# konstantineder/montecarlo-risk-engine

Hardware: AMD Instinct MI355X
Metric: path-steps/sec at 1M paths x 250 steps; PV/CVA rel-error vs CPU ref (higher is better)
Workload: dtype f64

## Files before the change

### montecarlo-risk-engine_amd/csrc/kf_lean.hip

```cpp
#include <cstdlib>
#include <map>
#include <utility>

#include "kf_common.h"

namespace {

template <int NSLOT, int PPL>
__device__ __forceinline__ void lean_date_cva(const FastDateCvaLds* __restrict__ rp, const double (&reg)[PPL][2 * NSLOT], double (&cva)[PPL],
                                              const double* __restrict__ etab)
{
    const mcx_expq_coef ec = mcx_expq_load(mcx_region_zero());
    const FastDateCvaLds r = *rp;
    double xe[2 * PPL], ev[2 * PPL];
#pragma unroll
    for (int q = 0; q < PPL; ++q) {
        xe[2 * q] = fma(r.m_s1, reg[q][FDC_S_REG], fma(r.m_n1, reg[q][FDC_NI_REG], r.m_c0));
        xe[2 * q + 1] = fma(r.c_c1, reg[q][FDC_C_REG], r.c_c0);
    }
    mcx_exp_tab_n<2 * PPL>(xe, ev, etab, ec);
#pragma unroll
    for (int q = 0; q < PPL; ++q) {
        const double x = fma(r.x_d, reg[q][FDC_X_REG], r.x_a);
        double p = 0.0;
        p += fma(fma(r.row0[2], x, r.row0[1]), x, r.row0[0]);
        p += fma(fma(r.row1[2], x, r.row1[1]), x, r.row1[0]);
        const double w = r.m_b * ev[2 * q];
        const double cs = fma(r.c_b, ev[2 * q + 1], r.c_a);
        cva[q] = fma(fmax(p, 0.0), w * (1.0 - cs), cva[q]);
    }
}

#define MCX_LEAN_WAVES 4
template <int NSLOT, int NZ, bool INJECT, int SIG, int PPL, bool SIMULATE, int DK = 0>
__global__ __launch_bounds__(MCX_BLOCK, MCX_LEAN_WAVES) void kf_lean(const FusedArgs)
{
    static_assert(DK == 0 || (SIG == SIG_VAS_CIR_E && SIMULATE && !INJECT), "the cva-date kernel simulates the Vasicek + CIR++ signature");
    constexpr int NREG = 2 * NSLOT;
    constexpr int TILE = MCX_BLOCK * PPL;
    extern __shared__ double lds[];
    KArgs& a0 = kargs_region(0);
    const int n_rec = a0.n_rec;
    const int64_t n = a0.k1.n;
    for (int q = threadIdx.x; q < 9 * n_rec; q += MCX_BLOCK) lds[q] = 0.0;
    FastDateCvaLds* const dlds = (FastDateCvaLds*)(lds + ((9 * n_rec + 1) & ~1));
    if constexpr (DK == 1) {
        const FastDateCva* __restrict__ dc = a0.cva_dates;
        const double* __restrict__ cf = a0.coeffs;
        const int n_dates = a0.n_dates;
        for (int q = threadIdx.x; q < 16 * n_dates; q += MCX_BLOCK) {
            const int t = q >> 4, e = q & 15;
            double v;
            if (e < FDC_HEAD) {
                v = ((const double*)(dc + t))[e];
            } else {
                const int off = e < FDC_HEAD + 3 ? dc[t].coeff_off0 : dc[t].coeff_off1;
                v = off >= 0 ? cf[off + (e - FDC_HEAD) % 3] : 0.0;
            }
            ((double*)dlds)[q] = v;
        }
    }
    constexpr int BMB = SIG == SIG_VAS_CIR_E ? 10 : 7;
    constexpr int BM = (INJECT || !SIMULATE) ? 0 : MCX_BM_LDS_DOUBLES_B(BMB);
    __shared__ double tab_lds[BM + MCX_EXP_LDS_DOUBLES];
    const double* tab = nullptr;
    const double* etab = tab_lds + BM;
    mcx_exp_tab_load(tab_lds + BM);
    if (BM) { mcx_bm_load<BMB>(tab_lds); tab = tab_lds; }
    __syncthreads();
    const int64_t tiles = (n + TILE - 1) / TILE;
    double n_block = 0.0;

    for (int64_t tile = blockIdx.x; tile < tiles; tile += gridDim.x) {
        const bool first_tile = tile == (int64_t)blockIdx.x;
        int64_t i[PPL];
        bool live[PPL];
        uint64_t path[PPL];
        double reg[PPL][NREG];
        double cfs[PPL], cva[PPL];
        int est[PPL];
        int n_init, n_steps;
        {
            KArgs& a = kargs_region(mcx_region_zero());
            const auto& k = a.k1;
#pragma unroll
            for (int q = 0; q < PPL; ++q) {
                const int64_t i_raw = tile * TILE + q * MCX_BLOCK + threadIdx.x;
                live[q] = i_raw < n;
                i[q] = live[q] ? i_raw : n - 1;
                path[q] = k.path_offset + (uint64_t)i[q];
                sim_init_state<NSLOT, SIG>(k, reg[q]);
                cfs[q] = 0.0; cva[q] = 0.0;
                est[q] = a.init_state[0];
            }
            const int64_t rest = n - tile * TILE;
            n_block += (double)(rest < TILE ? rest : TILE);
            n_init = k.n_initial_store; n_steps = k.n_steps;
        }
        if (SIMULATE) {
        int step = 0, t_init = 0;
#pragma unroll 1
        while (true) {
            const bool init = t_init < n_init;
            if (!init && step >= n_steps) break;
            int st = init ? t_init : -1;
            t_init += init ? 1 : 0;
            {
                const int zr0 = mcx_region_zero();
                const auto& k = kargs_region(zr0).k1;
                const uint64_t seed = k.seed;
                const mcx_bm_coef bc = mcx_bm_coef_load(zr0);
                const mcx_bm_vconst vc = mcx_bm_vconst_make<BMB>(bc);
#pragma unroll 1
                while (st < 0 && step < n_steps) {
                    if constexpr (SIG == SIG_GENERIC) {
#pragma unroll
                        for (int q = 0; q < PPL; ++q) sim_substep<NSLOT, NZ, INJECT, SIG, BMB, true>(k, step, path[q], i[q], reg[q], tab, seed, bc, &vc);
                        st = ldk(&k.steps[step].store_idx);
                    } else {
                        double zz[PPL][NZ], uu[PPL];
                        bool rare = false;
                        const StepData<NSLOT, NZ> sdat = sim_step_load<NSLOT, NZ, SIG>(k, step);
                        __builtin_amdgcn_sched_barrier(0);
                        if constexpr (INJECT) {
#pragma unroll
                            for (int q = 0; q < PPL; ++q) sim_draw<NZ, true, SIG, BMB>(k, step, path[q], i[q], zz[q], uu[q], tab, seed, bc, &vc);
                        } else {
                            uint32_t st_q[PPL];
#pragma unroll
                            for (int q = 0; q < PPL; ++q) st_q[q] = (uint32_t)step;
                            rare = sim_draw_n<PPL, NZ, SIG, BMB>(k, st_q, path, zz, uu, tab, seed, bc, vc);
                        }
                        if (!INJECT && __builtin_expect(__any(rare), 0)) {
#pragma unroll
                            for (int q = 0; q < PPL; ++q) sim_draw<NZ, false, SIG, BMB, true>(k, step, path[q], i[q], zz[q], uu[q], tab, seed, bc, &vc);
                        }
#pragma unroll
                        for (int q = 0; q < PPL; ++q) st = sim_apply_loaded<NSLOT, NZ, SIG, true>(k, sdat, reg[q], zz[q], uu[q]);
                    }
                    ++step;
                }
            }
            if (st >= 0) {
                if constexpr (DK == 1) lean_date_cva<NSLOT, PPL>(dlds + st, reg, cva, etab);
                else lean_date<NSLOT, SIG, PPL, true>(st, i, live, first_tile, lds, reg, cfs, cva, est, etab);
            }
        }
        } else {
            auto load_row = [&](int t, double (&dst)[PPL][NREG]) {
                const auto& k = kargs_region(0).k1;
                const int D = k.n_state;
#pragma unroll
                for (int q = 0; q < PPL; ++q)
#pragma unroll
                    for (int sl = 0; sl < NSLOT; ++sl) {
                        const bool bs = sig_kind(SIG, sl) >= 0 ? sig_is_bs(SIG, sl) : (k.slots[sl].kind == MCX_MODEL_BS);
                        const int c = k.slots[sl].state_off;
                        dst[q][2 * sl] = k.paths[((int64_t)t * D + c) * k.ld + i[q]];
                        dst[q][2 * sl + 1] = bs ? 0.0 : k.paths[((int64_t)t * D + c + 1) * k.ld + i[q]];
                    }
            };
            const int n_dates = kargs_region(0).n_dates;
            double bufb[PPL][NREG];
            load_row(0, reg);
            load_row(n_dates > 1 ? 1 : 0, bufb);
#pragma unroll 1
            for (int t = 0; t < n_dates; t += 2) {
                lean_date<NSLOT, SIG, PPL, false>(t, i, live, first_tile, lds, reg, cfs, cva, est, etab);
                if (t + 2 < n_dates) load_row(t + 2, reg);
                if (t + 1 < n_dates) {
                    lean_date<NSLOT, SIG, PPL, false>(t + 1, i, live, first_tile, lds, bufb, cfs, cva, est, etab);
                    if (t + 3 < n_dates) load_row(t + 3, bufb);
                }
            }
        }
        {
            KArgs& a = kargs_region(mcx_region_zero());
#pragma unroll
            for (int q = 0; q < PPL; ++q) if (a.cfs && live[q]) a.cfs[i[q]] = cfs[q];
            if (a.rec_pv[0] >= 0) lean_record<PPL>(cfs, live, a.rec_pv[0], n_rec, first_tile, lds);
            if (a.rec_cva[0] >= 0) {
                const double lgd = a.lgd[0];
                double cc[PPL];
#pragma unroll
                for (int q = 0; q < PPL; ++q) cc[q] = cva[q] * lgd;
                lean_record<PPL>(cc, live, a.rec_cva[0], n_rec, first_tile, lds);
            }
        }
    }
    __syncthreads();
    for (int r = threadIdx.x; r < n_rec; r += MCX_BLOCK) {
        double s1 = 0.0, s2 = 0.0;
        for (int w = 0; w < 4; ++w) { s1 += lds[n_rec + (w * n_rec + r) * 2]; s2 += lds[n_rec + (w * n_rec + r) * 2 + 1]; }
        double* dst = a0.partials + ((int64_t)blockIdx.x * n_rec + r) * 4;
        dst[0] = n_block; dst[1] = lds[r]; dst[2] = s1; dst[3] = s2;
    }
}

template <int NSLOT, int NZ, int SIG, int PPL>
int launch_lean_shape(const FusedArgs& a, int n_cu, bool inject, bool simulate, hipStream_t s)
{
    const int64_t tiles = (a.k1.n + MCX_BLOCK * PPL - 1) / (MCX_BLOCK * PPL);
    const size_t lds = sizeof(double) * (size_t)((9 * a.n_rec + 1) & ~1);
    const size_t lds_cva = lds + sizeof(FastDateCvaLds) * (size_t)a.n_dates;
    auto residency = [&](auto kernel, size_t bytes) {
        thread_local std::map<std::pair<const void*, size_t>, int> cache;
        const auto key = std::make_pair((const void*)kernel, bytes);
        auto it = cache.find(key);
        if (it == cache.end()) {
            int per_cu = 0;
            if (hipOccupancyMaxActiveBlocksPerMultiprocessor(&per_cu, kernel, MCX_BLOCK, bytes) != hipSuccess || per_cu < 1) per_cu = 1;
            it = cache.emplace(key, per_cu < MCX_LEAN_WAVES ? per_cu : MCX_LEAN_WAVES).first;
        }
        return (int64_t)it->second * n_cu;
    };
    auto sized = [&](int64_t resident) {
        if (tiles <= resident) return (int)tiles;
        const int64_t per = (tiles + resident - 1) / resident;
// ... 79 lines not shown
```

### montecarlo-risk-engine_amd/csrc/mcx_device.h

```cpp
#pragma once
#include "mcx_internal.h"

struct K1Args {
    mcx_slot slots[MCX_MAX_SLOTS];
    double init_state[MCX_MAX_STATE];
    const mcx_step* __restrict__ steps;
    const double* __restrict__ chol;
    const double* __restrict__ aux;
    double* __restrict__ paths;
    const double* __restrict__ inject_z;
    const double* __restrict__ inject_u;
    const double* __restrict__ init_paths;
    int64_t n, ld;
    uint64_t seed, path_offset;
    int32_t scheme, n_steps, n_state, n_initial_store, flags, n_uniform;
};

static inline void mcx_fill_k1_args(const mcx_sim* sim, uint64_t seed, uint64_t path_offset, int64_t n_paths, int64_t ld,
                                    double* d_paths, const double* d_inject_z, const double* d_inject_u, K1Args* a)
{
    const mcx_sim_desc& d = sim->desc;
    memset(a, 0, sizeof(*a));
    for (int s = 0; s < d.n_slots; ++s) a->slots[s] = d.slots[s];
    for (int c = 0; c < d.n_state; ++c) a->init_state[c] = d.init_state[c];
    a->steps = sim->d_steps; a->chol = sim->d_chol; a->aux = sim->d_aux;
    a->paths = d_paths; a->inject_z = d_inject_z; a->inject_u = d_inject_u;
    a->n = n_paths; a->ld = ld; a->seed = seed; a->path_offset = path_offset;
    a->scheme = d.scheme; a->n_steps = d.n_steps; a->n_state = d.n_state; a->n_initial_store = d.n_initial_store;
    a->flags = d.flags; a->n_uniform = d.n_uniform;
}

__device__ __forceinline__ void philox4x32_10(uint32_t c0, uint32_t c1, uint32_t c2, uint32_t c3, uint32_t k0, uint32_t k1,
                                              uint32_t& o0, uint32_t& o1, uint32_t& o2, uint32_t& o3)
{
#pragma unroll
    for (int r = 0; r < 10; ++r) {
        const uint64_t p0 = (uint64_t)0xD2511F53u * c0;
        const uint64_t p1 = (uint64_t)0xCD9E8D57u * c2;
        const uint32_t n0 = __builtin_amdgcn_bitop3_b32((uint32_t)(p1 >> 32), c1, k0, 0x96);
        const uint32_t n2 = __builtin_amdgcn_bitop3_b32((uint32_t)(p0 >> 32), c3, k1, 0x96);
        c1 = (uint32_t)p1;
        c3 = (uint32_t)p0;
        c0 = n0;
        c2 = n2;
        k0 += 0x9E3779B9u;
        k1 += 0xBB67AE85u;
    }
    o0 = c0; o1 = c1; o2 = c2; o3 = c3;
}

__device__ __forceinline__ double u53(uint32_t lo, uint32_t hi, const mcx_bm_vconst* vc = nullptr)
{
    if (vc) return fma((double)hi, vc->s32, fma((double)(lo >> 11), vc->s53, vc->c54));
    return fma((double)hi, 0x1.0p-32, fma((double)(lo >> 11), 0x1.0p-53, 0x1.0p-54));
}

struct DevBridge {
    uint64_t seed, path_offset;
    const double* const* inject;
    int64_t ld;
};

__device__ __forceinline__ double dev_barrier_event(const DevEvent& e, const DevTerm* __restrict__ terms, const double* __restrict__ coeffs,
                                                    const DevBridge* __restrict__ bridge, const double* __restrict__ paths, int64_t D,
                                                    int64_t ld, int64_t i, double num)
{
    const int types = (int)e.aux[3];
    const int t1 = types & 7, t2 = types >> 3;
    const bool with_bridge = e.aux[0] == 5.0;
    double mx = -1.0e300, mn = 1.0e300, keep1 = 1.0, keep2 = 1.0, prev1 = 0.0, prev2 = 0.0;
    double c = 0.0;
    int draw_id = 0;
    DevBridge br = {0, 0, nullptr, 0};
    const double* __restrict__ inj = nullptr;
    if (with_bridge) {
        c = ldk(coeffs + e.coeff_off);
        draw_id = (int)ldk(coeffs + e.coeff_off + 1);
        br = ldk_struct(bridge);
        if (br.inject) inj = br.inject[draw_id];
    }
    AtomCache bc = {-1, -1, 0.0};
    for (int j = e.term_begin; j < e.term_end; ++j) {
        const double s = dev_atom_cached(ldk_struct(&terms[j]).atom, paths, D, ld, i, bc);
        mx = fmax(mx, s); mn = fmin(mn, s);
        if (with_bridge) {
            const double cur1 = mcx_log(s / e.aux[1]), cur2 = t2 ? mcx_log(s / e.aux[2]) : 0.0;
            if (j > e.term_begin) {
                const int k = j - e.term_begin - 1;
                for (int bi = 0; bi < (t2 ? 2 : 1); ++bi) {
                    const double p = mcx_exp(c * (bi ? prev2 * cur2 : prev1 * cur1));
                    double u;
                    if (inj) u = inj[(int64_t)(2 * k + bi) * br.ld + i];
                    else {
                        uint32_t w0, w1, w2, w3;
                        const uint64_t path = br.path_offset + (uint64_t)i;
                        philox4x32_10((uint32_t)path, (uint32_t)(path >> 32), (uint32_t)k, 0x80000000u | (uint32_t)(2 * draw_id + bi),
                                      (uint32_t)br.seed, (uint32_t)(br.seed >> 32), w0, w1, w2, w3);
                        u = u53(w0, w1);
                    }
                    const double hit = fmin(fmax((p - u + 0.05) / 0.1, 0.0), 1.0);
                    if (bi) keep2 *= 1.0 - hit; else keep1 *= 1.0 - hit;
                }
            }
            prev1 = cur1; prev2 = cur2;
        }
    }
    double pay = fmax(e.sign * (dev_atom(e.x, paths, D, ld, i) - e.strike), 0.0) * dev_barrier_ind(t1, e.aux[1], mx, mn);
    if (with_bridge) pay *= (t1 <= 2) ? keep1 : 1.0 - keep1;
    if (t2) {
        pay *= dev_barrier_ind(t2, e.aux[2], mx, mn);
        if (with_bridge) pay *= (t2 <= 2) ? keep2 : 1.0 - keep2;
    }
    return pay / num;
}

template <bool TAB = false, int BMB = 7, bool GUARD = true>
__device__ __forceinline__ bool pair_from_words(uint32_t w0, uint32_t w1, uint32_t w2, uint32_t w3, double& ua, double& z0, double& z1,
                                                const double* __restrict__ tab, const mcx_bm_coef& bc, const mcx_bm_vconst* vc = nullptr)
{
    ua = u53(w0, w1, vc);
    double s, c, r;
    if (TAB) {
        const double r2 = mcx_m2log_tab<BMB>(ua, tab, bc, vc);
        if (!GUARD) r = mcx_sqrt_gp(r2);
        else if (__builtin_expect(__any(w1 == 0xffffffffu), 0)) r = ua < 1.0 ? mcx_sqrt_g(r2) : 0.0;
        else r = mcx_sqrt_gp(r2);
        const int j = (int)(w3 >> (32 - BMB));
        const double ur = u53(w2, w3 & ((1u << (32 - BMB)) - 1u), vc);
        mcx_sincos2pi_tab<BMB>(ur, j, tab, s, c, bc, vc);
    } else {
        r = mcx_sqrt(-2.0 * mcx_log(ua));
        mcx_sincos2pi(u53(w2, w3), s, c);
    }
    z0 = r * c;
    z1 = r * s;
    return w1 == 0xffffffffu;
}

template <bool TAB = false, int BMB = 7, bool GUARD = true>
__device__ __forceinline__ bool draw_pair(uint64_t seed, uint64_t path, uint32_t step, uint32_t draw, double& ua, double& z0, double& z1,
                                          const double* __restrict__ tab, const mcx_bm_coef& bc, const mcx_bm_vconst* vc = nullptr)
{
    uint32_t w0, w1, w2, w3;
    philox4x32_10((uint32_t)path, (uint32_t)(path >> 32), step, draw, (uint32_t)seed, (uint32_t)(seed >> 32), w0, w1, w2, w3);
    return pair_from_words<TAB, BMB, GUARD>(w0, w1, w2, w3, ua, z0, z1, tab, bc, vc);
}

template <bool TAB = false>
__device__ __forceinline__ void draw_pair(uint64_t seed, uint64_t path, uint32_t step, uint32_t draw, double& ua, double& z0, double& z1,
                                          const double* __restrict__ tab = nullptr)
{
    const mcx_bm_coef bc = mcx_bm_coef_load();
    draw_pair<TAB>(seed, path, step, draw, ua, z0, z1, tab, bc);
}

__device__ __forceinline__ double degree_of_truth(double x, bool fuzzy, double eps)
{
    if (!fuzzy) return x > 0.0 ? 1.0 : 0.0;
    const double v = (x + eps) / (2.0 * eps);
    return fmin(fmax(v, 0.0), 1.0);
}

struct AuxPtr {
    const double* __restrict__ p;
    __device__ __forceinline__ double operator[](int i) const { return ldk(p + i); }
    __device__ __forceinline__ mcx_aux_drv drv() const { return ldk_struct((const mcx_aux_drv*)(p + MCX_AUX_C0)); }
};
struct AuxRegs {
    double v[MCX_AUX];
    __device__ __forceinline__ double operator[](int i) const { return v[i]; }
    __device__ __forceinline__ mcx_aux_drv drv() const { mcx_aux_drv d; d.c0 = v[MCX_AUX_C0]; d.c1 = v[MCX_AUX_C1]; d.c2 = v[MCX_AUX_C2]; return d; }
};

template <int KIND, int SCHEME, bool POS = false, class SL, class AUX>
__device__ __forceinline__ void step_slot(const SL& sl, int scheme_rt, int flags, double dt, double sq,
                                          const AUX& aux, double& s0, double& s1, double zc0, double zc1, double u)
{
    const auto* p = sl.p;
    const int scheme = SCHEME >= 0 ? SCHEME : scheme_rt;
    switch (KIND >= 0 ? KIND : sl.kind) {
    case MCX_MODEL_BS:
        if (scheme == MCX_SCHEME_ANALYTICAL) {
            s0 = s0 * mcx_exp(aux[0] + (zc0 - aux[1]));
        } else {
            const mcx_aux_drv dc = aux.drv();
            s0 = fma(s0, fma(dc.c2, zc0, dc.c0), s0);
        }
        break;
    case MCX_MODEL_VASICEK: {
        const double r = s0;
        s1 = s1 + r * dt;
        if (scheme == MCX_SCHEME_ANALYTICAL) s0 = (p[2] + (r - p[2]) * aux[0]) + zc0;
        else {
            const mcx_aux_drv dc = aux.drv();
            s0 = fma(dc.c1, r, s0);
            s0 = fma(dc.c2, zc0, s0);
            s0 = s0 + dc.c0;
        }
        break;
    }
    case MCX_MODEL_HW: {
        const double r = s0;
        s1 = s1 + r * dt;
        if (scheme == MCX_SCHEME_ANALYTICAL) s0 = r * aux[0] + aux[1] + zc0;
        else s0 = r + (aux[0] - p[3] * r) * dt + p[1] * sq * zc0;
        break;
    }
    case MCX_MODEL_CIRPP: {
        const double y = s0;
        const double sy = POS ? mcx_sqrt_gp(y) : mcx_sqrt_g(y);
        const mcx_aux_drv dc = aux.drv();
        s1 = fma(y + aux[0], dt, s1);
        s0 = fma(dc.c1, y, s0);
        s0 = fma(dc.c2 * sy, zc0, s0);
        s0 = s0 + dc.c0;
        s0 = fmax(s0, 1e-12);
        break;
    }
    case MCX_MODEL_CIRPP_DET:
        s1 = s1 + aux[0] * dt;
        s0 = aux[1];
        break;
    case MCX_MODEL_S2F: {
        const double x = s0, y = s1;
        if (scheme == MCX_SCHEME_ANALYTICAL) {
            s0 = x * aux[0] + zc0;
            s1 = y + p[3] * dt + zc1;
        } else {
            s0 = x - p[1] * x * dt + p[2] * sq * zc0;
            s1 = y + p[3] * dt + p[4] * sq * zc1;
        }
        break;
    }
    case MCX_MODEL_HESTON: {
        const double logS = s0, v = s1;
        const double sigma = p[1], rate = p[2], kappa = p[4], theta = p[5];
        if (scheme == MCX_SCHEME_EULER) {
            const double sv = mcx_sqrt(fmax(v, 0.0));
            s0 = logS + (rate - 0.5 * v) * dt + sv * sq * zc0;
            s1 = fmax(v + kappa * (theta - v) * dt + sigma * sv * sq * zc1, 0.0);
        } else {
            const double eps = 1e-12;
            const bool fuzzy = (flags & MCX_FLAG_SMOOTHING) != 0;
            const double m = theta + (v - theta) * aux[0];
            const double s2 = v * aux[6] + aux[7];
            const double omu = fmax(1.0 - u, eps);
            const double d1 = m * m + eps, d5 = m + eps;
            const double d15 = d1 * d5;
            const double ra = mcx_rcp(d15 * omu);
            const double r_omu = ra * d15, ra6 = ra * omu;
            const double r1 = ra6 * d5, r5 = ra6 * d1;
            const double psi = s2 * r1;
            const double d2 = psi + eps, d4 = psi + 1.0;
            const double rb = mcx_rcp(d2 * d4);
            const double invpsi = rb * d4, r4 = rb * d2;
            const double t = fmax(2.0 * invpsi - 1.0, 0.0);
            double root = mcx_sqrt_g(2.0 * invpsi * t);
            root = invpsi < 0.0 ? __builtin_nan("") : root;
            const double b2u = 2.0 * invpsi - 1.0 + root;
            const double b2 = b2u < 0.0 ? 0.0 : b2u;
            const double b = mcx_sqrt_g(b2);
            const double pp = fmin(fmax((psi - 1.0) * r4, 0.0), 1.0 - 1e-6);
            const double beta = (1.0 - pp) * r5;
            const double d3 = 1.0 + b2, d7 = beta + eps;
            const double rc = mcx_rcp(d3 * d7);
            const double a = m * (rc * d7);
            const double v1 = a * (b + zc1) * (b + zc1);
            const double omp = fmax(1.0 - pp, eps);
            const double v_tail = mcx_log(omp * r_omu) * (rc * d3);
            const double v2 = degree_of_truth(u - pp, fuzzy, 0.3) * v_tail;
            const double w = degree_of_truth(psi - 1.5, fuzzy, 0.5);
            const double vn = (1.0 - w) * v1 + w * v2;
            const double var_int = fmax(aux[4] * v + aux[5] * vn, 0.0);
            const double vol = mcx_sqrt_gp(fmax(var_int, eps));
            s0 = logS + rate * dt + aux[1] + aux[2] * v + aux[3] * vn + vol * zc0;
            s1 = vn;
        }
        break;
    }
    default: break;
    }
}


enum { SIG_GENERIC = 0, SIG_VAS_CIR_E = 1, SIG_BS_A = 2, SIG_BS_E = 3, SIG_HESTON_QE = 4, SIG_HESTON_E = 5,
       SIG_VAS_E = 6, SIG_VAS_A = 7, SIG_BS_VAS_CIRDET_E = 8 };

__host__ __device__ constexpr int sig_kind(int sig, int slot)
{
    return sig == SIG_VAS_CIR_E ? (slot == 0 ? MCX_MODEL_VASICEK : MCX_MODEL_CIRPP)
         : (sig == SIG_BS_A || sig == SIG_BS_E) ? MCX_MODEL_BS
         : (sig == SIG_HESTON_QE || sig == SIG_HESTON_E) ? MCX_MODEL_HESTON
         : (sig == SIG_VAS_E || sig == SIG_VAS_A) ? MCX_MODEL_VASICEK
         : sig == SIG_BS_VAS_CIRDET_E ? (slot == 0 ? MCX_MODEL_BS : slot == 1 ? MCX_MODEL_VASICEK : MCX_MODEL_CIRPP_DET)
         : -1;
}
__host__ __device__ constexpr int sig_scheme(int sig)
{
    return (sig == SIG_VAS_CIR_E || sig == SIG_BS_E || sig == SIG_HESTON_E || sig == SIG_VAS_E || sig == SIG_BS_VAS_CIRDET_E) ? MCX_SCHEME_EULER
         : (sig == SIG_BS_A || sig == SIG_VAS_A) ? MCX_SCHEME_ANALYTICAL
         : sig == SIG_HESTON_QE ? MCX_SCHEME_QE : -1;
}
__host__ __device__ constexpr bool sig_is_bs(int sig, int slot) { return sig_kind(sig, slot) == MCX_MODEL_BS; }

static inline int mcx_sim_signature(const mcx_sim_desc& d)
{
    auto k = [&](int s) { return d.slots[s].kind; };
    if (d.n_slots == 2 && k(0) == MCX_MODEL_VASICEK && k(1) == MCX_MODEL_CIRPP && d.scheme == MCX_SCHEME_EULER) return SIG_VAS_CIR_E;
    if (d.n_slots == 3 && k(0) == MCX_MODEL_BS && k(1) == MCX_MODEL_VASICEK && k(2) == MCX_MODEL_CIRPP_DET && d.scheme == MCX_SCHEME_EULER)
        return SIG_BS_VAS_CIRDET_E;
    if (d.n_slots == 1) {
        if (k(0) == MCX_MODEL_BS) return d.scheme == MCX_SCHEME_ANALYTICAL ? SIG_BS_A : d.scheme == MCX_SCHEME_EULER ? SIG_BS_E : SIG_GENERIC;
        if (k(0) == MCX_MODEL_HESTON) return d.scheme == MCX_SCHEME_QE ? SIG_HESTON_QE : d.scheme == MCX_SCHEME_EULER ? SIG_HESTON_E : SIG_GENERIC;
        if (k(0) == MCX_MODEL_VASICEK) return d.scheme == MCX_SCHEME_EULER ? SIG_VAS_E : d.scheme == MCX_SCHEME_ANALYTICAL ? SIG_VAS_A : SIG_GENERIC;
    }
    return SIG_GENERIC;
}

__device__ __forceinline__ AuxPtr aux_of_slot(const double* __restrict__ ax, int s) { return AuxPtr{ax + s * MCX_AUX}; }
template <int NSLOT>
__device__ __forceinline__ const AuxRegs& aux_of_slot(const AuxRegs (&ax)[NSLOT], int s) { return ax[s]; }

template <int NSLOT, int NZ, int SIG, int S, bool POS = false, class KA, class AX>
__device__ __forceinline__ void step_slots(const KA& k, const mcx_step& sp, const AX& ax,
                                           double (&reg)[2 * NSLOT], const double (&zc)[NZ], double u)
{
    if constexpr (S < NSLOT) {
        const double zc0 = (NSLOT == 1) ? zc[0] : zc[S < NZ ? S : 0];
        const double zc1 = (NSLOT == 1 && NZ > 1) ? zc[NZ > 1 ? 1 : 0] : 0.0;
        step_slot<sig_kind(SIG, S), sig_scheme(SIG), POS>(k.slots[S], k.scheme, k.flags | k.slots[S].flags, sp.dt, sp.sqrt_dt,
                                                      aux_of_slot(ax, S), reg[2 * S], reg[2 * S + 1], zc0, zc1, u);
        step_slots<NSLOT, NZ, SIG, S + 1, POS>(k, sp, ax, reg, zc, u);
    }
}

template <int NZ, bool INJECT, int SIG, int BMB = 7, bool GUARD = true, class KA>
__device__ __forceinline__ bool sim_draw(const KA& k, int step, uint64_t path, int64_t i, double (&z)[NZ], double& u,
                                         const double* __restrict__ tab, uint64_t seed, const mcx_bm_coef& bc, const mcx_bm_vconst* vc = nullptr)
{
    u = 0.0;
    bool rare = false;
    if (INJECT) {
#pragma unroll
        for (int j = 0; j < NZ; ++j) z[j] = k.inject_z[((int64_t)step * NZ + j) * k.ld + i];
        if (k.n_uniform) u = k.inject_u[(int64_t)step * k.ld + i];
    } else {
        double ua;
#pragma unroll
        for (int q = 0; q < (NZ + 1) / 2; ++q) {
            double z0, z1;
            rare |= draw_pair<true, BMB, GUARD>(seed, path, (uint32_t)step, (uint32_t)q, ua, z0, z1, tab, bc, vc);
            z[2 * q] = z0;
            if (2 * q + 1 < NZ) z[2 * q + 1] = z1;
        }
        if (sig_scheme(SIG) == MCX_SCHEME_QE || (sig_scheme(SIG) < 0 && k.n_uniform)) {
            double z0, z1;
            draw_pair<false>(seed, path, (uint32_t)step, (uint32_t)((NZ + 1) / 2), u, z0, z1, nullptr, bc);
        }
    }
    return rare;
}

template <int PPL>
__device__ __forceinline__ void philox4x32_10_n(const uint64_t (&path)[PPL], const uint32_t (&step)[PPL], uint32_t draw, uint64_t seed,
                                                uint32_t (&o0)[PPL], uint32_t (&o1)[PPL], uint32_t (&o2)[PPL], uint32_t (&o3)[PPL])
{
    uint32_t c0[PPL], c1[PPL], c2[PPL], c3[PPL];
#pragma unroll
    for (int q = 0; q < PPL; ++q) { c0[q] = (uint32_t)path[q]; c1[q] = (uint32_t)(path[q] >> 32); c2[q] = step[q]; c3[q] = draw; }
    uint32_t k0 = (uint32_t)seed, k1 = (uint32_t)(seed >> 32);
#pragma unroll
    for (int r = 0; r < 10; ++r) {
#pragma unroll
        for (int q = 0; q < PPL; ++q) {
            const uint64_t p0 = (uint64_t)0xD2511F53u * c0[q];
            const uint64_t p1 = (uint64_t)0xCD9E8D57u * c2[q];
            const uint32_t n0 = __builtin_amdgcn_bitop3_b32((uint32_t)(p1 >> 32), c1[q], k0, 0x96);
            const uint32_t n2 = __builtin_amdgcn_bitop3_b32((uint32_t)(p0 >> 32), c3[q], k1, 0x96);
            c1[q] = (uint32_t)p1; c3[q] = (uint32_t)p0; c0[q] = n0; c2[q] = n2;
        }
        k0 += 0x9E3779B9u;
        k1 += 0xBB67AE85u;
    }
#pragma unroll
    for (int q = 0; q < PPL; ++q) { o0[q] = c0[q]; o1[q] = c1[q]; o2[q] = c2[q]; o3[q] = c3[q]; }
}

template <int PPL, int BMB>
__device__ __forceinline__ bool draw_pairs_staged(uint64_t seed, const uint64_t (&path)[PPL], const uint32_t (&step)[PPL], uint32_t draw,
                                                  double (&z0)[PPL], double (&z1)[PPL], const double* __restrict__ tab,
                                                  const mcx_bm_coef& C, const mcx_bm_vconst& vc)
{
    constexpr int N = 1 << BMB, LOG_TERMS = mcx_bm_shape<BMB>::LOG_TERMS;
    uint32_t w0[PPL], w1[PPL], w2[PPL], w3[PPL];
    philox4x32_10_n<PPL>(path, step, draw, seed, w0, w1, w2, w3);
    double m[PPL], ed[PPL], ps[PPL], pc[PPL];
    int e[PPL];
    mcx_d2 tc[PPL], sc[PPL];
#pragma unroll
    for (int q = 0; q < PPL; ++q) {
        const double ua = u53(w0[q], w1[q], &vc);
        m[q] = __builtin_amdgcn_frexp_mant(ua);
        e[q] = __builtin_amdgcn_frexp_exp(ua);
        const int jl = (__double2hiint(m[q]) >> (20 - BMB)) & (N - 1);
        tc[q] = ((const mcx_d2*)tab)[jl];
        sc[q] = ((const mcx_d2*)(tab + 2 * N))[(int)(w3[q] >> (32 - BMB))];
    }
    __builtin_amdgcn_sched_barrier(0);
#pragma unroll
    for (int q = 0; q < PPL; ++q) {
        const double ur = u53(w2[q], w3[q] & ((1u << (32 - BMB)) - 1u), &vc);
        const double d = fma(ur, 6.28318530717958647692, vc.trig_off);
        const double d2 = d * d;
        double qs, qc;
        if constexpr (mcx_bm_shape<BMB>::TRIG_TERMS == 3) {
            qs = fma(fma(vc.sin_head, d2, C.c[7]), d2, C.c[6]);
            qc = fma(fma(vc.cos_head, d2, C.c[10]), d2, C.c[9]);
        } else {
            qs = fma(vc.sin_head, d2, C.c[6]);
            qc = fma(vc.cos_head, d2, C.c[9]);
        }
        ps[q] = fma(d * d2, qs, d);
        pc[q] = fma(d2, qc, 1.0);
        ed[q] = (double)e[q];
    }
    __builtin_amdgcn_sched_barrier(0);
    bool rare = false;
#pragma unroll
    for (int q = 0; q < PPL; ++q) {
        const double s = fma(m[q], tc[q].x, 2.0);
        double p = vc.log_head;
#pragma unroll
        for (int k = LOG_TERMS - 2; k >= 0; --k) p = fma(p, s, C.c[k]);
        const double r2 = fma(ed[q], -2.0 * 6.93147180559945309417e-01, tc[q].y) + fma(s * s, p, s);
        const double r = mcx_sqrt_gp(r2);
        const double sn = fma(sc[q].x, pc[q], sc[q].y * ps[q]);
        const double cs = fma(-sc[q].x, ps[q], sc[q].y * pc[q]);
        z0[q] = r * cs;
        z1[q] = r * sn;
        rare |= w1[q] == 0xffffffffu;
    }
    return rare;
}

template <int PPL, int NZ, int SIG, int BMB, class KA>
__device__ __forceinline__ bool sim_draw_n(const KA& k, const uint32_t (&step)[PPL], const uint64_t (&path)[PPL], double (&z)[PPL][NZ], double (&u)[PPL],
                                           const double* __restrict__ tab, uint64_t seed, const mcx_bm_coef& bc, const mcx_bm_vconst& vc)
{
    bool rare = false;
#pragma unroll
    for (int dq = 0; dq < (NZ + 1) / 2; ++dq) {
        double a[PPL], b[PPL];
        rare |= draw_pairs_staged<PPL, BMB>(seed, path, step, (uint32_t)dq, a, b, tab, bc, vc);
#pragma unroll
        for (int q = 0; q < PPL; ++q) { z[q][2 * dq] = a[q]; if (2 * dq + 1 < NZ) z[q][2 * dq + 1] = b[q]; }
    }
#pragma unroll
    for (int q = 0; q < PPL; ++q) {
        u[q] = 0.0;
        if (sig_scheme(SIG) == MCX_SCHEME_QE || (sig_scheme(SIG) < 0 && k.n_uniform)) {
            double t0, t1;
            draw_pair<false>(seed, path[q], step[q], (uint32_t)((NZ + 1) / 2), u[q], t0, t1, nullptr, bc);
        }
    }
    return rare;
}

template <int NSLOT, int NZ, int SIG, bool POS = false, class KA>
__device__ __forceinline__ int sim_apply(const KA& k, int step, double (&reg)[2 * NSLOT], const double (&z)[NZ], double u)
{
    const mcx_step sp = ldk_struct(&k.steps[step]);
    double zc[NZ];
    constexpr bool UNIT_L00 = sig_scheme(SIG) == MCX_SCHEME_EULER || sig_scheme(SIG) == MCX_SCHEME_QE;
    const double* __restrict__ L = UNIT_L00 ? k.chol : k.chol + (int64_t)sp.chol_idx * NZ * NZ;
#pragma unroll
    for (int r = 0; r < NZ; ++r) {
        double acc = (UNIT_L00 && r == 0) ? z[0] : ldk(L + r * NZ) * z[0];
#pragma unroll
        for (int c = 1; c <= r; ++c) acc = fma(ldk(L + r * NZ + c), z[c], acc);
        zc[r] = acc;
    }
    const double* __restrict__ ax = k.aux + (int64_t)step * NSLOT * MCX_AUX;
    step_slots<NSLOT, NZ, SIG, 0, POS>(k, sp, ax, reg, zc, u);
    return sp.store_idx;
}

template <int NSLOT, int NZ>
struct StepData {
    mcx_step sp;
    double L[NZ * NZ];
    AuxRegs ax[NSLOT];
};
template <int NSLOT, int NZ, int SIG, class KA>
__device__ __forceinline__ StepData<NSLOT, NZ> sim_step_load(const KA& k, int step)
{
    StepData<NSLOT, NZ> d;
    d.sp = ldk_struct(&k.steps[step]);
    constexpr bool UNIT_L00 = sig_scheme(SIG) == MCX_SCHEME_EULER || sig_scheme(SIG) == MCX_SCHEME_QE;
    const double* __restrict__ L = UNIT_L00 ? k.chol : k.chol + (int64_t)d.sp.chol_idx * NZ * NZ;
#pragma unroll
    for (int q = 0; q < NZ * NZ; ++q) d.L[q] = ldk(L + q);
    struct P2 { double v[2]; };
    struct P4 { double v[4]; };
    static_assert(MCX_AUX == 8, "aux row layout");
    const double* __restrict__ ax = k.aux + (int64_t)step * NSLOT * MCX_AUX;
#pragma unroll
    for (int s = 0; s < NSLOT; ++s) {
        const P2 a = ldk_struct((const P2*)(ax + s * MCX_AUX)), b = ldk_struct((const P2*)(ax + s * MCX_AUX + 2));
        const P4 c = ldk_struct((const P4*)(ax + s * MCX_AUX + 4));
        d.ax[s].v[0] = a.v[0]; d.ax[s].v[1] = a.v[1]; d.ax[s].v[2] = b.v[0]; d.ax[s].v[3] = b.v[1];
#pragma unroll
        for (int q = 0; q < 4; ++q) d.ax[s].v[4 + q] = c.v[q];
    }
    return d;
}
template <int NSLOT, int NZ, int SIG, bool POS = false, class KA>
__device__ __forceinline__ int sim_apply_loaded(const KA& k, const StepData<NSLOT, NZ>& d, double (&reg)[2 * NSLOT], const double (&z)[NZ], double u)
{
    double zc[NZ];
    constexpr bool UNIT_L00 = sig_scheme(SIG) == MCX_SCHEME_EULER || sig_scheme(SIG) == MCX_SCHEME_QE;
#pragma unroll
    for (int r = 0; r < NZ; ++r) {
        double acc = (UNIT_L00 && r == 0) ? z[0] : d.L[r * NZ] * z[0];
#pragma unroll
        for (int c = 1; c <= r; ++c) acc = fma(d.L[r * NZ + c], z[c], acc);
        zc[r] = acc;
    }
    step_slots<NSLOT, NZ, SIG, 0, POS>(k, d.sp, d.ax, reg, zc, u);
    return d.sp.store_idx;
}

template <int NSLOT, int NZ, bool INJECT, int SIG, int BMB = 7, bool POS = false, class KA>
__device__ __forceinline__ void sim_substep(const KA& k, int step, uint64_t path, int64_t i, double (&reg)[2 * NSLOT],
                                            const double* __restrict__ tab, uint64_t seed, const mcx_bm_coef& bc, const mcx_bm_vconst* vc = nullptr)
{
    double z[NZ], u;
// ... 47 lines not shown
```

### montecarlo-risk-engine_amd/csrc/mcx_math.h

```cpp
#pragma once

__device__ const double MCX_EXP_C[14] __attribute__((aligned(64))) = {1.00000000000000000e+00, 1.00000000000000000e+00, 5.00000000000000000e-01, 1.66666666666666657e-01, 4.16666666666666644e-02, 8.33333333333333322e-03, 1.38888888888888894e-03, 1.98412698412698413e-04, 2.48015873015873016e-05, 2.75573192239858925e-06, 2.75573192239858883e-07, 2.50521083854417202e-08, 2.08767569878681002e-09, 1.60590438368216133e-10};
__device__ const double MCX_SIN_C[10] = {3.14159265358979312e+00, -5.16771278004997026e+00, 2.55016403987734552e+00, -5.99264529320792105e-01, 8.21458866111282326e-02, -7.37043094571435044e-03, 4.66302805767612554e-04, -2.19153534478302173e-05, 7.95205400147551261e-07, -2.29484289972698730e-08};
__device__ const double MCX_COS_C[10] = {1.00000000000000000e+00, -4.93480220054467900e+00, 4.05871212641676848e+00, -1.33526276885458950e+00, 2.35330630358893206e-01, -2.58068913900140612e-02, 1.92957430940392314e-03, -1.04638104924845705e-04, 4.30306958703294729e-06, -1.38789524622137714e-07};
__device__ const double MCX_LOG_C[7] = {6.666666666666735130e-01, 3.999999999940941908e-01, 2.857142874366239149e-01, 2.222219843214978396e-01, 1.818357216161805012e-01, 1.531383769920937332e-01, 1.479819860511658591e-01};

__device__ __forceinline__ int mcx_region_zero()
{
    int z;
    asm volatile("s_mov_b32 %0, 0" : "=s"(z));
    return z;
}
__device__ __forceinline__ uint32_t mcx_region_copy(uint32_t v)
{
    uint32_t o;
    asm volatile("s_mov_b32 %0, %1" : "=s"(o) : "s"(v));
    return o;
}

struct mcx_exp_coef { double c[14]; };
__device__ __forceinline__ mcx_exp_coef mcx_exp_load(int z = 0)
{
    return ldk_struct((const mcx_exp_coef*)(MCX_EXP_C + z));
}
// ... 30 lines not shown
    double rr = __builtin_amdgcn_rcp(dd);
    rr = fma(fma(-dd, rr, 1.0), rr, rr);
    rr = fma(fma(-dd, rr, 1.0), rr, rr);
    double s = f * rr;
    s = fma(fma(-dd, s, f), rr, s);
    const double z = s * s;
    double R = ldk(MCX_LOG_C + 6);
#pragma unroll
    for (int j = 5; j >= 0; --j) R = fma(R, z, ldk(MCX_LOG_C + j));
    R *= z;
    const double hfsq = 0.5 * f * f;
    const double dk = (double)e;
    return dk * 6.93147180369123816490e-01 - ((hfsq - (s * (hfsq + R) + dk * 1.90821492927058770002e-10)) - f);
}

__device__ __forceinline__ void mcx_sincos2pi(double u, double& s, double& c)
{
    const double x = u + u;
    const double n = rint(x + x);
    const double r = fma(n, -0.5, x);
    const double t = r * r;
    double ps = ldk(MCX_SIN_C + 9), pc = ldk(MCX_COS_C + 9);
#pragma unroll
    for (int j = 8; j >= 0; --j) { ps = fma(ps, t, ldk(MCX_SIN_C + j)); pc = fma(pc, t, ldk(MCX_COS_C + j)); }
    ps *= r;
    const int q = (int)n;
    const bool swap = q & 1;
    const double a = swap ? pc : ps, b = swap ? ps : pc;
    s = (q & 2) ? -a : a;
    c = ((q + 1) & 2) ? -b : b;
}

__device__ __forceinline__ double mcx_rcp(double d)
{
    double r = __builtin_amdgcn_rcp(d);
    r = fma(fma(-d, r, 1.0), r, r);
    r = fma(fma(-d, r, 1.0), r, r);
    return r;
}

__device__ __forceinline__ double mcx_sqrt(double a)
{
    const double y = __builtin_amdgcn_rsq(a);
    double g = a * y, h = 0.5 * y;
    const double r = fma(-h, g, 0.5);
    g = fma(g, r, g);
    h = fma(h, r, h);
    const double d = fma(-g, g, a);
    g = fma(d, h, g);
    return a > 0.0 ? g : 0.0;
}

__device__ __forceinline__ double mcx_sqrt_h(double a, double& h_out)
{
    const double y = __builtin_amdgcn_rsq(a);
    double g = a * y, h = 0.5 * y;
    const double r = fma(-h, g, 0.5);
    g = fma(g, r, g);
    h = fma(h, r, h);
    const double d = fma(-g, g, a);
    g = fma(d, h, g);
    h_out = a <= 0.0 ? __builtin_huge_val() : h;
    return a <= 0.0 ? 0.0 : g;
}

__device__ __forceinline__ double mcx_sqrt_g(double a)
{
    const double y = __builtin_amdgcn_rsq(a);
    double g = a * y;
    const double h = 0.5 * y;
    const double r = fma(-h, g, 0.5);
    g = fma(g, r, g);
    return a <= 0.0 ? 0.0 : g;
}

__device__ __forceinline__ double mcx_sqrt_gp(double a)
{
    const double y = __builtin_amdgcn_rsq(a);
    const double g = a * y;
    const double h = 0.5 * y;
    return fma(g, fma(-h, g, 0.5), g);
}

#include "mcx_tables.h"
#define MCX_BM_LDS_DOUBLES_B(BMB) (4 << (BMB))
#define MCX_BM_LDS_DOUBLES MCX_BM_LDS_DOUBLES_B(7)
template <int BMB> struct mcx_bm_shape;
template <> struct mcx_bm_shape<7> {
    static constexpr int LOG_TERMS = 6, TRIG_TERMS = 3;
    static __device__ __forceinline__ double log_src(int q) { return MCX_LOG_TAB[q]; }
    static __device__ __forceinline__ double trig_src(int q) { return MCX_TRIG_TAB[q]; }
};
template <> struct mcx_bm_shape<10> {
    static constexpr int LOG_TERMS = 4, TRIG_TERMS = 2;
    static __device__ __forceinline__ double log_src(int q) { return MCX_LOG_TAB_L[q]; }
    static __device__ __forceinline__ double trig_src(int q) { return MCX_TRIG_TAB_L[q]; }
};

__device__ const double MCX_BM_C[12] __attribute__((aligned(64))) = {0.25, (1.0 / 3.0) * 0.25, 0.03125, 0.2 * 0.0625, (1.0 / 6.0) * 0.03125, (1.0 / 7.0) * 0.015625,
                                                                     -1.0 / 6.0, 1.0 / 120.0, -1.0 / 5040.0, -0.5, 1.0 / 24.0, -1.0 / 720.0};
struct mcx_bm_coef { double c[12]; };
__device__ __forceinline__ mcx_bm_coef mcx_bm_coef_load(int z = 0)
{
    return ldk_struct((const mcx_bm_coef*)(MCX_BM_C + z));
}

struct mcx_bm_vconst {
    double c54;
    double s53, s32;
    double log_head;
    double sin_head, cos_head;
    double trig_off;
};
__device__ __forceinline__ double mcx_opaque_v(double x) { asm volatile("" : "+v"(x)); return x; }
__device__ __forceinline__ double mcx_opaque_s(double x) { asm volatile("" : "+s"(x)); return x; }
template <int BMB = 7>
__device__ __forceinline__ mcx_bm_vconst mcx_bm_vconst_make(const mcx_bm_coef& C)
{
    using SH = mcx_bm_shape<BMB>;
    mcx_bm_vconst v;
    v.c54 = mcx_opaque_v(0x1.0p-54); v.s53 = mcx_opaque_s(0x1.0p-53); v.s32 = mcx_opaque_s(0x1.0p-32);
    v.log_head = mcx_opaque_v(C.c[SH::LOG_TERMS - 1]);
    v.sin_head = mcx_opaque_v(C.c[5 + SH::TRIG_TERMS]);
    v.cos_head = mcx_opaque_v(C.c[8 + SH::TRIG_TERMS]);
    v.trig_off = mcx_opaque_v(-3.14159265358979323846 / (double)(1 << BMB));
    return v;
}

template <int BMB = 7>
__device__ __forceinline__ void mcx_bm_load(double* __restrict__ tab)
{
    constexpr int N = 1 << BMB;
    for (int q = threadIdx.x; q < 2 * N; q += blockDim.x) {
        tab[q] = -2.0 * mcx_bm_shape<BMB>::log_src(q);
        tab[2 * N + q] = mcx_bm_shape<BMB>::trig_src(q);
    }
    __syncthreads();
}

typedef double mcx_d2 __attribute__((ext_vector_type(2)));

template <int BMB = 7>
__device__ __forceinline__ double mcx_m2log_tab(double x, const double* __restrict__ tab, const mcx_bm_coef& C, const mcx_bm_vconst* vc = nullptr)
{
    constexpr int N = 1 << BMB, LOG_TERMS = mcx_bm_shape<BMB>::LOG_TERMS;
    const double m = __builtin_amdgcn_frexp_mant(x);
    const int e = __builtin_amdgcn_frexp_exp(x);
    const int j = (__double2hiint(m) >> (20 - BMB)) & (N - 1);
    const mcx_d2 tc = ((const mcx_d2*)tab)[j];
    const double s = fma(m, tc.x, 2.0);
    double q = vc ? vc->log_head : C.c[LOG_TERMS - 1];
#pragma unroll
    for (int k = LOG_TERMS - 2; k >= 0; --k) q = fma(q, s, C.c[k]);
    const double p = fma(s * s, q, s);
    return fma((double)e, -2.0 * 6.93147180559945309417e-01, tc.y) + p;
}

template <int BMB = 7>
__device__ __forceinline__ void mcx_sincos2pi_tab(double ur, int j, const double* __restrict__ tab, double& s, double& c, const mcx_bm_coef& C,
                                                  const mcx_bm_vconst* vc = nullptr)
{
    constexpr int N = 1 << BMB;
    const double d = fma(ur, 6.28318530717958647692, vc ? vc->trig_off : -3.14159265358979323846 / (double)N);
    const mcx_d2 sc = ((const mcx_d2*)(tab + 2 * N))[j];
    const double d2 = d * d;
    double qs, qc;
    if constexpr (mcx_bm_shape<BMB>::TRIG_TERMS == 3) {
        qs = fma(fma(vc ? vc->sin_head : C.c[8], d2, C.c[7]), d2, C.c[6]);
        qc = fma(fma(vc ? vc->cos_head : C.c[11], d2, C.c[10]), d2, C.c[9]);
    } else {
        qs = fma(vc ? vc->sin_head : C.c[7], d2, C.c[6]);
        qc = fma(vc ? vc->cos_head : C.c[10], d2, C.c[9]);
    }
    const double ps = fma(d * d2, qs, d);
    const double pc = fma(d2, qc, 1.0);
    s = fma(sc.x, pc, sc.y * ps);
    c = fma(-sc.x, ps, sc.y * pc);
}

#define MCX_EXP_LDS_DOUBLES 128
__device__ const double MCX_EXPQ_C[4] __attribute__((aligned(32))) = {0.5, 1.0 / 6.0, 1.0 / 24.0, 1.0 / 120.0};
struct mcx_expq_coef { double c[4]; };
__device__ __forceinline__ mcx_expq_coef mcx_expq_load(int z = 0) { return ldk_struct((const mcx_expq_coef*)(MCX_EXPQ_C + z)); }

__device__ __forceinline__ void mcx_exp_tab_load(double* __restrict__ tab)
{
    for (int q = threadIdx.x; q < MCX_EXP_LDS_DOUBLES; q += blockDim.x) tab[q] = MCX_EXP2_TAB[q];
}

__device__ __forceinline__ double mcx_exp_tab(double x, const double* __restrict__ tab, const mcx_expq_coef& C)
{
    const double k = rint(x * MCX_128_LN2);
    double r = fma(k, -MCX_LN2_128_HI, x);
    r = fma(k, -MCX_LN2_128_LO, r);
    const int ki = (int)k;
    const double T = tab[ki & 127];
    double q = fma(C.c[3], r, C.c[2]);
    q = fma(q, r, C.c[1]);
    q = fma(q, r, C.c[0]);
    q = fma(q, r, 1.0);
    q *= r;
    return ldexp(fma(T, q, T), ki >> 7);
}

// ... 27 lines not shown
```

Before: 292.0 billion.

## Shave integer and FP ops from Philox and Box-Muller in VAS_CIR_E lean path

For the VAS_CIR_E PPL=2 simulate path, the change precomputes the first three Philox rounds when the high path word is warp-uniform, so it is passed as a scalar. It also builds uniforms by bit-packing into the double mantissa instead of using int-to-double conversions, and takes the exponent and table index straight from the raw bits. Sqrt refinement now negates the half-reciprocal through exponent-bit arithmetic rather than an FP multiply. The goal is fewer VALU instructions per normal draw, at the cost of extra per-lane constant registers and subtle bit-level correctness risks.

After: 303.3 billion (median of 6 runs). +3.9%, better.

```diff
diff --git a/montecarlo-risk-engine_amd/csrc/kf_lean.hip b/montecarlo-risk-engine_amd/csrc/kf_lean.hip
--- a/montecarlo-risk-engine_amd/csrc/kf_lean.hip
+++ b/montecarlo-risk-engine_amd/csrc/kf_lean.hip
@@ -62,6 +62,7 @@
     }
     constexpr int BMB = SIG == SIG_VAS_CIR_E ? 10 : 7;
     constexpr int BM = (INJECT || !SIMULATE) ? 0 : MCX_BM_LDS_DOUBLES_B(BMB);
+    constexpr bool FLOOR = SIG == SIG_VAS_CIR_E && PPL == 2 && SIMULATE && !INJECT;
     __shared__ double tab_lds[BM + MCX_EXP_LDS_DOUBLES];
     const double* tab = nullptr;
     const double* etab = tab_lds + BM;
@@ -80,6 +81,8 @@
         double cfs[PPL], cva[PPL];
         int est[PPL];
         int n_init, n_steps;
+        bool uhi = false;
+        uint32_t hs = 0;
         {
             KArgs& a = kargs_region(mcx_region_zero());
             const auto& k = a.k1;
@@ -96,6 +99,7 @@
             const int64_t rest = n - tile * TILE;
             n_block += (double)(rest < TILE ? rest : TILE);
             n_init = k.n_initial_store; n_steps = k.n_steps;
+            if (FLOOR) uhi = philox_uniform_hi<PPL>(path, hs);
         }
         if (SIMULATE) {
         int step = 0, t_init = 0;
@@ -110,7 +114,7 @@
                 const auto& k = kargs_region(zr0).k1;
                 const uint64_t seed = k.seed;
                 const mcx_bm_coef bc = mcx_bm_coef_load(zr0);
-                const mcx_bm_vconst vc = mcx_bm_vconst_make<BMB>(bc);
+                const mcx_bm_vconst vc = mcx_bm_vconst_make<BMB, FLOOR>(bc);
 #pragma unroll 1
                 while (st < 0 && step < n_steps) {
                     if constexpr (SIG == SIG_GENERIC) {
@@ -129,11 +133,12 @@
                             uint32_t st_q[PPL];
 #pragma unroll
                             for (int q = 0; q < PPL; ++q) st_q[q] = (uint32_t)step;
-                            rare = sim_draw_n<PPL, NZ, SIG, BMB>(k, st_q, path, zz, uu, tab, seed, bc, vc);
+                            if (FLOOR && uhi) rare = sim_draw_n<PPL, NZ, SIG, BMB, FLOOR, true>(k, st_q, path, zz, uu, tab, seed, bc, vc, hs);
+                            else rare = sim_draw_n<PPL, NZ, SIG, BMB, FLOOR, false>(k, st_q, path, zz, uu, tab, seed, bc, vc);
                         }
                         if (!INJECT && __builtin_expect(__any(rare), 0)) {
 #pragma unroll
-                            for (int q = 0; q < PPL; ++q) sim_draw<NZ, false, SIG, BMB, true>(k, step, path[q], i[q], zz[q], uu[q], tab, seed, bc, &vc);
+                            for (int q = 0; q < PPL; ++q) sim_draw<NZ, false, SIG, BMB, true>(k, step, path[q], i[q], zz[q], uu[q], tab, seed, bc, FLOOR ? nullptr : &vc);
                         }
 #pragma unroll
                         for (int q = 0; q < PPL; ++q) st = sim_apply_loaded<NSLOT, NZ, SIG, true>(k, sdat, reg[q], zz[q], uu[q]);
diff --git a/montecarlo-risk-engine_amd/csrc/mcx_device.h b/montecarlo-risk-engine_amd/csrc/mcx_device.h
--- a/montecarlo-risk-engine_amd/csrc/mcx_device.h
+++ b/montecarlo-risk-engine_amd/csrc/mcx_device.h
@@ -53,6 +53,21 @@
 {
     if (vc) return fma((double)hi, vc->s32, fma((double)(lo >> 11), vc->s53, vc->c54));
     return fma((double)hi, 0x1.0p-32, fma((double)(lo >> 11), 0x1.0p-53, 0x1.0p-54));
+}
+
+__device__ __forceinline__ double u53_nocvt(uint32_t lo, uint32_t hi, const mcx_bm_vconst& vc, int q = 0)
+{
+    return fma((double)hi, vc.s32, __hiloint2double((int)vc.hi_half[q & 1], (int)(lo >> 11)) + vc.c54h);
+}
+
+template <int BMB>
+__device__ __forceinline__ double u53_rem(uint32_t lo, uint32_t hi, const mcx_bm_vconst& vc)
+{
+    uint32_t f;
+    asm("v_bfe_u32 %0, %1, 11, %2" : "=v"(f) : "v"(hi), "n"(21 - BMB));
+    const uint32_t h = 0x43300000u | f;
+    const uint32_t l = (hi << 21) | (lo >> 11);
+    return fma(__hiloint2double((int)h, (int)l), vc.s53, vc.c54h);
 }
 
 struct DevBridge {
@@ -208,7 +223,7 @@
     }
     case MCX_MODEL_CIRPP: {
         const double y = s0;
-        const double sy = POS ? mcx_sqrt_gp(y) : mcx_sqrt_g(y);
+        const double sy = POS ? mcx_sqrt_gpi(y) : mcx_sqrt_g(y);
         const mcx_aux_drv dc = aux.drv();
         s1 = fma(y + aux[0], dt, s1);
         s0 = fma(dc.c1, y, s0);
@@ -362,54 +377,95 @@
 }
 
 template <int PPL>
+__device__ __forceinline__ bool philox_uniform_hi(const uint64_t (&path)[PPL], uint32_t& hs)
+{
+    hs = __builtin_amdgcn_readfirstlane((uint32_t)(path[0] >> 32));
+    bool same = true;
+#pragma unroll
+    for (int q = 0; q < PPL; ++q) same = same && (uint32_t)(path[q] >> 32) == hs;
+    return __all(same) != 0;
+}
+
+template <int PPL, bool UHI = false>
 __device__ __forceinline__ void philox4x32_10_n(const uint64_t (&path)[PPL], const uint32_t (&step)[PPL], uint32_t draw, uint64_t seed,
-                                                uint32_t (&o0)[PPL], uint32_t (&o1)[PPL], uint32_t (&o2)[PPL], uint32_t (&o3)[PPL])
-{
+                                                uint32_t (&o0)[PPL], uint32_t (&o1)[PPL], uint32_t (&o2)[PPL], uint32_t (&o3)[PPL], uint32_t hs = 0)
+{
+    constexpr uint32_t M0 = 0xD2511F53u, M1 = 0xCD9E8D57u, W0 = 0x9E3779B9u, W1 = 0xBB67AE85u;
     uint32_t c0[PPL], c1[PPL], c2[PPL], c3[PPL];
 #pragma unroll
     for (int q = 0; q < PPL; ++q) { c0[q] = (uint32_t)path[q]; c1[q] = (uint32_t)(path[q] >> 32); c2[q] = step[q]; c3[q] = draw; }
     uint32_t k0 = (uint32_t)seed, k1 = (uint32_t)(seed >> 32);
-#pragma unroll
-    for (int r = 0; r < 10; ++r) {
+    int r0 = 0;
+    if constexpr (UHI) {
 #pragma unroll
         for (int q = 0; q < PPL; ++q) {
-            const uint64_t p0 = (uint64_t)0xD2511F53u * c0[q];
-            const uint64_t p1 = (uint64_t)0xCD9E8D57u * c2[q];
+            const uint64_t a0 = (uint64_t)M0 * c0[q], a1 = (uint64_t)M1 * c2[q];
+            const uint32_t s0 = (uint32_t)(a1 >> 32) ^ hs ^ k0;
+            const uint32_t v2 = __builtin_amdgcn_bitop3_b32((uint32_t)(a0 >> 32), c3[q], k1, 0x96);
+            const uint32_t s1 = (uint32_t)a1, v3 = (uint32_t)a0;
+            const uint64_t b0 = (uint64_t)M0 * s0, b1 = (uint64_t)M1 * v2;
+            const uint32_t v0 = (uint32_t)(b1 >> 32) ^ (s1 ^ (k0 + W0));
+            const uint32_t v2b = v3 ^ ((uint32_t)(b0 >> 32) ^ (k1 + W1));
+            const uint32_t v1 = (uint32_t)b1, s3 = (uint32_t)b0;
+            const uint64_t d0 = (uint64_t)M0 * v0, d1 = (uint64_t)M1 * v2b;
+            c0[q] = __builtin_amdgcn_bitop3_b32((uint32_t)(d1 >> 32), v1, k0 + 2 * W0, 0x96);
+            c2[q] = (uint32_t)(d0 >> 32) ^ (s3 ^ (k1 + 2 * W1));
+            c1[q] = (uint32_t)d1; c3[q] = (uint32_t)d0;
+        }
+        k0 += 3 * W0; k1 += 3 * W1;
+        r0 = 3;
+    }
+#pragma unroll
+    for (int r = r0; r < 10; ++r) {
+#pragma unroll
+        for (int q = 0; q < PPL; ++q) {
+            const uint64_t p0 = (uint64_t)M0 * c0[q];
+            const uint64_t p1 = (uint64_t)M1 * c2[q];
             const uint32_t n0 = __builtin_amdgcn_bitop3_b32((uint32_t)(p1 >> 32), c1[q], k0, 0x96);
             const uint32_t n2 = __builtin_amdgcn_bitop3_b32((uint32_t)(p0 >> 32), c3[q], k1, 0x96);
             c1[q] = (uint32_t)p1; c3[q] = (uint32_t)p0; c0[q] = n0; c2[q] = n2;
         }
-        k0 += 0x9E3779B9u;
-        k1 += 0xBB67AE85u;
+        k0 += W0;
+        k1 += W1;
     }
 #pragma unroll
     for (int q = 0; q < PPL; ++q) { o0[q] = c0[q]; o1[q] = c1[q]; o2[q] = c2[q]; o3[q] = c3[q]; }
 }
 
-template <int PPL, int BMB>
+template <int PPL, int BMB, bool FLOOR = false, bool UHI = false>
 __device__ __forceinline__ bool draw_pairs_staged(uint64_t seed, const uint64_t (&path)[PPL], const uint32_t (&step)[PPL], uint32_t draw,
                                                   double (&z0)[PPL], double (&z1)[PPL], const double* __restrict__ tab,
-                                                  const mcx_bm_coef& C, const mcx_bm_vconst& vc)
-{
+                                                  const mcx_bm_coef& C, const mcx_bm_vconst& vc, uint32_t hs = 0)
+{
+    static_assert(!FLOOR || PPL <= 2, "one high-word register per path of a lane (mcx_bm_vconst)");
     constexpr int N = 1 << BMB, LOG_TERMS = mcx_bm_shape<BMB>::LOG_TERMS;
     uint32_t w0[PPL], w1[PPL], w2[PPL], w3[PPL];
-    philox4x32_10_n<PPL>(path, step, draw, seed, w0, w1, w2, w3);
+    philox4x32_10_n<PPL, UHI>(path, step, draw, seed, w0, w1, w2, w3, hs);
     double m[PPL], ed[PPL], ps[PPL], pc[PPL];
+    uint32_t eb[PPL];
     int e[PPL];
     mcx_d2 tc[PPL], sc[PPL];
 #pragma unroll
     for (int q = 0; q < PPL; ++q) {
-        const double ua = u53(w0[q], w1[q], &vc);
-        m[q] = __builtin_amdgcn_frexp_mant(ua);
-        e[q] = __builtin_amdgcn_frexp_exp(ua);
-        const int jl = (__double2hiint(m[q]) >> (20 - BMB)) & (N - 1);
-        tc[q] = ((const mcx_d2*)tab)[jl];
+        if constexpr (FLOOR) {
+            const double ua = u53_nocvt(w0[q], w1[q], vc, q);
+            const uint32_t uh = (uint32_t)__double2hiint(ua);
+            eb[q] = uh >> 20;
+            m[q] = __builtin_amdgcn_frexp_mant(ua);
+            tc[q] = *(const mcx_d2*)((const char*)tab + ((uh >> (16 - BMB)) & ((N - 1) << 4)));
+        } else {
+            const double ua = u53(w0[q], w1[q], &vc);
+            m[q] = __builtin_amdgcn_frexp_mant(ua);
+            e[q] = __builtin_amdgcn_frexp_exp(ua);
+            const int jl = (__double2hiint(m[q]) >> (20 - BMB)) & (N - 1);
+            tc[q] = ((const mcx_d2*)tab)[jl];
+        }
         sc[q] = ((const mcx_d2*)(tab + 2 * N))[(int)(w3[q] >> (32 - BMB))];
     }
     __builtin_amdgcn_sched_barrier(0);
 #pragma unroll
     for (int q = 0; q < PPL; ++q) {
-        const double ur = u53(w2[q], w3[q] & ((1u << (32 - BMB)) - 1u), &vc);
+        const double ur = FLOOR ? u53_rem<BMB>(w2[q], w3[q], vc) : u53(w2[q], w3[q] & ((1u << (32 - BMB)) - 1u), &vc);
         const double d = fma(ur, 6.28318530717958647692, vc.trig_off);
         const double d2 = d * d;
         double qs, qc;
@@ -422,7 +478,8 @@
         }
         ps[q] = fma(d * d2, qs, d);
         pc[q] = fma(d2, qc, 1.0);
-        ed[q] = (double)e[q];
+        if constexpr (FLOOR) ed[q] = __hiloint2double((int)vc.hi_2p52[q & 1], (int)eb[q]) - (0x1.0p52 + 1022.0);
+        else ed[q] = (double)e[q];
     }
     __builtin_amdgcn_sched_barrier(0);
     bool rare = false;
@@ -433,7 +490,7 @@
 #pragma unroll
         for (int k = LOG_TERMS - 2; k >= 0; --k) p = fma(p, s, C.c[k]);
         const double r2 = fma(ed[q], -2.0 * 6.93147180559945309417e-01, tc[q].y) + fma(s * s, p, s);
-        const double r = mcx_sqrt_gp(r2);
+        const double r = FLOOR ? mcx_sqrt_gpi(r2) : mcx_sqrt_gp(r2);
         const double sn = fma(sc[q].x, pc[q], sc[q].y * ps[q]);
         const double cs = fma(-sc[q].x, ps[q], sc[q].y * pc[q]);
         z0[q] = r * cs;
@@ -443,15 +500,16 @@
     return rare;
 }
 
-template <int PPL, int NZ, int SIG, int BMB, class KA>
+template <int PPL, int NZ, int SIG, int BMB, bool FLOOR = false, bool UHI = false, class KA>
 __device__ __forceinline__ bool sim_draw_n(const KA& k, const uint32_t (&step)[PPL], const uint64_t (&path)[PPL], double (&z)[PPL][NZ], double (&u)[PPL],
-                                           const double* __restrict__ tab, uint64_t seed, const mcx_bm_coef& bc, const mcx_bm_vconst& vc)
+                                           const double* __restrict__ tab, uint64_t seed, const mcx_bm_coef& bc, const mcx_bm_vconst& vc,
+                                           uint32_t hs = 0)
 {
     bool rare = false;
 #pragma unroll
     for (int dq = 0; dq < (NZ + 1) / 2; ++dq) {
         double a[PPL], b[PPL];
-        rare |= draw_pairs_staged<PPL, BMB>(seed, path, step, (uint32_t)dq, a, b, tab, bc, vc);
+        rare |= draw_pairs_staged<PPL, BMB, FLOOR, UHI>(seed, path, step, (uint32_t)dq, a, b, tab, bc, vc, hs);
 #pragma unroll
         for (int q = 0; q < PPL; ++q) { z[q][2 * dq] = a[q]; if (2 * dq + 1 < NZ) z[q][2 * dq + 1] = b[q]; }
     }
diff --git a/montecarlo-risk-engine_amd/csrc/mcx_math.h b/montecarlo-risk-engine_amd/csrc/mcx_math.h
--- a/montecarlo-risk-engine_amd/csrc/mcx_math.h
+++ b/montecarlo-risk-engine_amd/csrc/mcx_math.h
@@ -136,6 +136,14 @@
     return fma(g, fma(-h, g, 0.5), g);
 }
 
+__device__ __forceinline__ double mcx_sqrt_gpi(double a)
+{
+    const double y = __builtin_amdgcn_rsq(a);
+    const double g = a * y;
+    const double mh = __hiloint2double((int)((uint32_t)__double2hiint(y) + 0x7FF00000u), __double2loint(y));
+    return fma(g, fma(mh, g, 0.5), g);
+}
+
 #include "mcx_tables.h"
 #define MCX_BM_LDS_DOUBLES_B(BMB) (4 << (BMB))
 #define MCX_BM_LDS_DOUBLES MCX_BM_LDS_DOUBLES_B(7)
@@ -161,19 +169,28 @@
 
 struct mcx_bm_vconst {
     double c54;
+    double c54h;
     double s53, s32;
     double log_head;
     double sin_head, cos_head;
     double trig_off;
+    uint32_t hi_half[2], hi_2p52[2];
 };
 __device__ __forceinline__ double mcx_opaque_v(double x) { asm volatile("" : "+v"(x)); return x; }
 __device__ __forceinline__ double mcx_opaque_s(double x) { asm volatile("" : "+s"(x)); return x; }
-template <int BMB = 7>
+__device__ __forceinline__ uint32_t mcx_opaque_v32(uint32_t x) { asm volatile("" : "+v"(x)); return x; }
+template <int BMB = 7, bool FLOOR = false>
 __device__ __forceinline__ mcx_bm_vconst mcx_bm_vconst_make(const mcx_bm_coef& C)
 {
     using SH = mcx_bm_shape<BMB>;
     mcx_bm_vconst v;
-    v.c54 = mcx_opaque_v(0x1.0p-54); v.s53 = mcx_opaque_s(0x1.0p-53); v.s32 = mcx_opaque_s(0x1.0p-32);
+    if (FLOOR) {
+        v.c54h = mcx_opaque_v(0x1.0p-54 - 0x1.0p-1);
+        for (int q = 0; q < 2; ++q) { v.hi_half[q] = mcx_opaque_v32(0x3FE00000u); v.hi_2p52[q] = mcx_opaque_v32(0x43300000u); }
+    } else {
+        v.c54 = mcx_opaque_v(0x1.0p-54);
+    }
+    v.s53 = mcx_opaque_s(0x1.0p-53); v.s32 = mcx_opaque_s(0x1.0p-32);
     v.log_head = mcx_opaque_v(C.c[SH::LOG_TERMS - 1]);
     v.sin_head = mcx_opaque_v(C.c[5 + SH::TRIG_TERMS]);
     v.cos_head = mcx_opaque_v(C.c[8 + SH::TRIG_TERMS]);
```
